# sykefi/syke-pic

Measured on AMD Instinct MI355X. Metric: IFCB images/sec, resnet50 224x224 infer step, higher is better.
Workload: dtype f16

## Files before the change

### syke-pic_amd/csrc/conv_stem.hip

```cpp
#include "spk_common.h"
#include <cstdlib>

namespace {

constexpr int TILE = 16;
constexpr int PH = 2 * TILE + 5;
constexpr int PWP = TILE + 4;
constexpr int PATCH_BYTES = PH * PWP * 16;
constexpr int W_ROW_BYTES = 512;

constexpr int POOL_STEP = 14;
constexpr int POOL_OUT = 7;

template <int DT, int SPLITW, int POOL>
__global__ __launch_bounds__(256) void conv_stem_kernel(ConvArgs a, int tiles_x, int tiles_y, int n_tiles) {
  constexpr int NW = SPLITW ? 2 : 1;
  constexpr int NJ = POOL ? 2 : 4;
  constexpr int WROWS = 16 * NJ;
  constexpr int W_BYTES = WROWS * W_ROW_BYTES;
  const int cb = POOL ? (int)(blockIdx.x & 1) : 0;
  constexpr int EPI_LD = 68;
  constexpr int TSTEP = POOL ? POOL_STEP : TILE;
  constexpr int TORG = POOL ? 1 : 0;
  extern __shared__ __attribute__((aligned(16))) unsigned char smem[];
  unsigned char* const sW = smem;
  unsigned char* const sP = smem + NW * W_BYTES;
  float* const sE = (float*)(sP + 2 * PATCH_BYTES);
  unsigned char* const sH = sP + 2 * PATCH_BYTES;
  constexpr int HSTRIDE = 80;

  const int tid = threadIdx.x, lane = tid & 63;
  const int wave = __builtin_amdgcn_readfirstlane(tid >> 6);
  const int frow = lane & 15, fq = lane >> 4;

  const __amdgpu_buffer_rsrc_t rx = __builtin_amdgcn_make_buffer_rsrc((void*)a.x, 0, a.x_bytes, 0x00020000);

  for (int c = tid; c < NW * WROWS * 32; c += 256) {
    const int ch = c & 31, row = (c >> 5) % WROWS, half = c / (WROWS * 32);
    const int srow = POOL ? 32 * cb + 8 * ((row & 15) >> 2) + 4 * (row >> 4) + (row & 3) : row;
    const u32x4_t v = *(const u32x4_t*)(a.w + ((size_t)(half * 64 + srow) * 256 + ch * 8));
    *(u32x4_t*)(sW + half * W_BYTES + row * W_ROW_BYTES + ((ch ^ (row & 15)) << 4)) = v;
  }

  constexpr int P_IT = (PH * PWP + 255) / 256;
  u32x4_t rp[P_IT];
  auto issue_patch = [&](int tile) {
    const int img = tile / (tiles_x * tiles_y);
    const int rem = tile - img * tiles_x * tiles_y;
    const int ty = rem / tiles_x, tx = rem - ty * tiles_x;
    const int iy0 = (ty * TSTEP - TORG) * 2 - 3, ix0 = (tx * TSTEP - TORG) * 2 - 4;
#pragma unroll
    for (int i = 0; i < P_IT; ++i) {
      const int c = tid + i * 256;
      const int pr = c / PWP, pp = c - pr * PWP;
      const int iy = iy0 + pr, ix = ix0 + 2 * pp;
      const bool ok = c < PH * PWP && (unsigned)iy < (unsigned)a.H && (unsigned)ix < (unsigned)a.W;
      const unsigned off = ok ? (unsigned)((((img * a.H + iy) * a.W) + ix) * 8) : 0x80000000u;
      rp[i] = __builtin_amdgcn_raw_buffer_load_b128(rx, off, 0, 0);
    }
  };
  auto store_patch = [&](int buf) {
#pragma unroll
    for (int i = 0; i < P_IT; ++i) {
      const int c = tid + i * 256;
      if (c < PH * PWP) *(u32x4_t*)(sP + buf * PATCH_BYTES + c * 16) = rp[i];
    }
  };

  const int ecol = (lane & 7) * 8, erow = lane >> 3;
  float sc[8], bi[8], s1[8], s2[8];
#pragma unroll
  for (int j = 0; j < 8; ++j) {
    sc[j] = a.scale ? a.scale[ecol + j] : 1.f;
    bi[j] = a.bias ? a.bias[ecol + j] : 0.f;
    s1[j] = s2[j] = 0.f;
  }
  float* const epi = sE + wave * (16 * EPI_LD);
  float psc[8], pbi[8];
  if (POOL) {
#pragma unroll
    for (int j = 0; j < 8; ++j) {
      psc[j] = a.scale ? a.scale[32 * cb + 8 * fq + j] : 1.f;
      pbi[j] = a.bias ? a.bias[32 * cb + 8 * fq + j] : 0.f;
    }
  }

  const int tstep = POOL ? (int)(gridDim.x >> 1) : (int)gridDim.x;
  int tile = POOL ? (int)(blockIdx.x >> 1) : (int)blockIdx.x;
  int buf = 0;
  if (tile < n_tiles) {
    issue_patch(tile);
    store_patch(0);
  }
  __syncthreads();
  for (; tile < n_tiles; tile += tstep) {
    const int next = tile + tstep;
    if (next < n_tiles) issue_patch(next);

    const int img = tile / (tiles_x * tiles_y);
    const int rem = tile - img * tiles_x * tiles_y;
    const int ty = rem / tiles_x, tx = rem - ty * tiles_x;
    const unsigned char* patch = sP + buf * PATCH_BYTES;

    f32x4_t acc[4][NJ];
#pragma unroll
    for (int i = 0; i < 4; ++i)
#pragma unroll
      for (int j = 0; j < NJ; ++j) acc[i][j] = f32x4_t{0.f, 0.f, 0.f, 0.f};
#pragma unroll
    for (int r = 0; r < 7; ++r) {
      u32x4_t fa[4], fb[NJ], fl[SPLITW ? NJ : 1];
#pragma unroll
      for (int i = 0; i < 4; ++i) {
        const int oy = wave * 4 + i;
        fa[i] = *(const u32x4_t*)(patch + ((2 * oy + r) * PWP + frow + fq) * 16);
      }
#pragma unroll
      for (int j = 0; j < NJ; ++j) {
        const int n = j * 16 + frow;
        fb[j] = *(const u32x4_t*)(sW + n * W_ROW_BYTES + (((r * 4 + fq) ^ (n & 15)) << 4));
        if (SPLITW) fl[j] = *(const u32x4_t*)(sW + W_BYTES + n * W_ROW_BYTES + (((r * 4 + fq) ^ (n & 15)) << 4));
      }
#pragma unroll
      for (int i = 0; i < 4; ++i)
#pragma unroll
        for (int j = 0; j < NJ; ++j) {
          if (POOL) {
            acc[i][j] = mfma16<DT>(fb[j], fa[i], acc[i][j]);
            if (SPLITW) acc[i][j] = mfma16<DT>(fl[j], fa[i], acc[i][j]);
          } else {
            acc[i][j] = mfma16<DT>(fa[i], fb[j], acc[i][j]);
            if (SPLITW) acc[i][j] = mfma16<DT>(fa[i], fl[j], acc[i][j]);
          }
        }
    }

    if (POOL) {
      typedef unsigned short u16x2_t __attribute__((ext_vector_type(2)));
      const int ox = tx * TSTEP - TORG + frow;
#pragma unroll
      for (int i = 0; i < 4; ++i) {
        const int oy = ty * TSTEP - TORG + wave * 4 + i;
        const bool inside = (unsigned)oy < (unsigned)a.Ho && (unsigned)ox < (unsigned)a.Wo;
        {
          u32x4_t ov = {0u, 0u, 0u, 0u};
          float v[8];
#pragma unroll
          for (int r = 0; r < 4; ++r) {
            v[r] = fmaxf(acc[i][0][r] * psc[r] + pbi[r], 0.f);
            v[4 + r] = fmaxf(acc[i][NJ - 1][r] * psc[4 + r] + pbi[4 + r], 0.f);
          }
          if (inside) {
#pragma unroll
            for (int j = 0; j < 4; ++j) ov[j] = pack2<DT>(v[2 * j], v[2 * j + 1]) & 0x7fff7fffu;
          }
          u32x4_t hm;
#pragma unroll
          for (int j = 0; j < 4; ++j) {
            unsigned own = ov[j];
            asm volatile("" : "+v"(own));
            unsigned n1 = (unsigned)__builtin_amdgcn_update_dpp(0, (int)own, 0x101, 0xf, 0xf, true);
            asm volatile("" : "+v"(n1), "+v"(own));
            const u16x2_t t = __builtin_elementwise_max(__builtin_bit_cast(u16x2_t, own), __builtin_bit_cast(u16x2_t, n1));
            unsigned n2 = (unsigned)__builtin_amdgcn_update_dpp(0, (int)n1, 0x101, 0xf, 0xf, true);
            asm volatile("" : "+v"(n2));
            const u16x2_t m = __builtin_elementwise_max(t, __builtin_bit_cast(u16x2_t, n2));
            hm[j] = __builtin_bit_cast(unsigned, m);
          }
          if (!(frow & 1) && frow < 2 * POOL_OUT)
            *(u32x4_t*)(sH + ((wave * 4 + i) * POOL_OUT + (frow >> 1)) * HSTRIDE + 8 * fq * 2) = hm;
        }
      }
    } else
#pragma unroll
    for (int i = 0; i < 4; ++i) {
#pragma unroll
      for (int j = 0; j < NJ; ++j)
#pragma unroll
        for (int rr = 0; rr < 4; ++rr) epi[(fq * 4 + rr) * EPI_LD + j * 16 + frow] = acc[i][j][rr];
      __builtin_amdgcn_wave_barrier();
      const int oy = ty * TSTEP - TORG + wave * 4 + i;
#pragma unroll
      for (int p = 0; p < 2; ++p) {
        const int px = erow + p * 8;
        const int ox = tx * TSTEP - TORG + px;
        const f32x4_t v0 = *(const f32x4_t*)(epi + px * EPI_LD + ecol);
        const f32x4_t v1 = *(const f32x4_t*)(epi + px * EPI_LD + ecol + 4);
        float v[8] = {v0[0], v0[1], v0[2], v0[3], v1[0], v1[1], v1[2], v1[3]};
        const bool inside = (unsigned)oy < (unsigned)a.Ho && (unsigned)ox < (unsigned)a.Wo;
        if (POOL) {
        } else if (inside) {
          if (a.stats) {
#pragma unroll
            for (int j = 0; j < 8; ++j) { s1[j] += v[j]; s2[j] += v[j] * v[j]; }
          }
#pragma unroll
          for (int j = 0; j < 8; ++j) {
            v[j] = v[j] * sc[j] + bi[j];
            if (a.relu) v[j] = fmaxf(v[j], 0.f);
          }
          u32x4_t ov;
#pragma unroll
          for (int j = 0; j < 4; ++j) ov[j] = pack2<DT>(v[2 * j], v[2 * j + 1]);
          *(u32x4_t*)(a.y + (((size_t)img * a.Ho + oy) * a.Wo + ox) * 64 + ecol) = ov;
        }
      }
      __builtin_amdgcn_wave_barrier();
    }

    if (next < n_tiles) store_patch(buf ^ 1);
    __syncthreads();
    if (POOL) {
      for (int it = tid; it < POOL_OUT * POOL_OUT * 4; it += 256) {
        const int chunk = it & 3, pp = it >> 2;
        const int ppy = pp / POOL_OUT, ppx = pp - ppy * POOL_OUT;
        const int py = ty * POOL_OUT + ppy, pxg = tx * POOL_OUT + ppx;
        if (py >= a.pool_ho || pxg >= a.pool_wo) continue;
        u32x4_t mx = {0u, 0u, 0u, 0u};
#pragma unroll
        for (int r = 0; r < 3; ++r) {
          const u32x4_t t = *(const u32x4_t*)(sH + ((2 * ppy + r) * POOL_OUT + ppx) * HSTRIDE + chunk * 16);
#pragma unroll
          for (int j = 0; j < 4; ++j) {
            const unsigned int av = mx[j], bv = t[j];
            const unsigned int lo = max(av & 0xffffu, bv & 0xffffu), hi = max(av >> 16, bv >> 16);
            mx[j] = lo | (hi << 16);
          }
        }
        *(u32x4_t*)(a.pool_y + (((size_t)img * a.pool_ho + py) * a.pool_wo + pxg) * 64 + 32 * cb + chunk * 8) = mx;
      }
      __syncthreads();
    }
    buf ^= 1;
  }

  if (a.stats) {
#pragma unroll
    for (int j = 0; j < 8; ++j)
      for (int d = 8; d < 64; d <<= 1) {
        s1[j] += __shfl_xor(s1[j], d);
        s2[j] += __shfl_xor(s2[j], d);
      }
    float* red = sE;
    __syncthreads();
    if (erow == 0) {
#pragma unroll
      for (int j = 0; j < 8; ++j) {
        red[(wave * 2 + 0) * 64 + ecol + j] = s1[j];
        red[(wave * 2 + 1) * 64 + ecol + j] = s2[j];
      }
    }
    __syncthreads();
    if (tid < 128) {
      const float t = (red[tid] + red[128 + tid]) + (red[256 + tid] + red[384 + tid]);
      a.stats[(size_t)blockIdx.x * 128 + tid] = t;
    }
  }
}

template <int DT, int SPLITW, int POOL>
int launch(const ConvArgs& a, hipStream_t s, int* m_tiles_out) {
  const int tiles_x = POOL ? (a.pool_wo + POOL_OUT - 1) / POOL_OUT : (a.Wo + TILE - 1) / TILE;
  const int tiles_y = POOL ? (a.pool_ho + POOL_OUT - 1) / POOL_OUT : (a.Ho + TILE - 1) / TILE;
  const int n_tiles = a.N * tiles_x * tiles_y;
  const size_t lds = (SPLITW ? 2 : 1) * (POOL ? 32 : 64) * W_ROW_BYTES + 2 * PATCH_BYTES +
                     (POOL ? TILE * POOL_OUT * 80 : 4 * 16 * 68 * 4);
  int grid = 256 * 2;
  if (SPLITW && !POOL) grid = 256;
  if (POOL) {
    if (grid > 2 * n_tiles) grid = 2 * n_tiles;
  } else if (grid > n_tiles) {
    grid = n_tiles;
  }
  auto k = conv_stem_kernel<DT, SPLITW, POOL>;
  static std::atomic<unsigned long long> attr;
  (void)spk_lds_limit_once(attr, (const void*)k, (int)lds);
  if (m_tiles_out) *m_tiles_out = grid;
  hipLaunchKernelGGL(k, dim3(grid), dim3(256), lds, s, a, tiles_x, tiles_y, n_tiles);
  return hipGetLastError() == hipSuccess ? 0 : -1;
}

}

int spk_conv_stem_launch(const ConvArgs& a, hipStream_t s, int* m_tiles_out) {
  if (a.Cout != 64 || a.kh != 7 || a.stride != 2 || a.pad != 3 || a.res) return -2;
  if (a.pool_y) {
    if (!a.relu || a.stats || a.pool_ho != (a.Ho - 1) / 2 + 1 || a.pool_wo != (a.Wo - 1) / 2 + 1) return -2;
    if (a.dt == DT_F16) return a.splitw ? launch<DT_F16, 1, 1>(a, s, m_tiles_out) : launch<DT_F16, 0, 1>(a, s, m_tiles_out);
    return launch<DT_BF16, 0, 1>(a, s, m_tiles_out);
  }
  if (a.dt == DT_F16) return a.splitw ? launch<DT_F16, 1, 0>(a, s, m_tiles_out) : launch<DT_F16, 0, 0>(a, s, m_tiles_out);
  return launch<DT_BF16, 0, 0>(a, s, m_tiles_out);
}
```

Before: 78410.

## Carry pooling halo across stem conv tiles instead of recomputing overlap

Adds a POOL==2 variant of the fused stem conv+maxpool kernel. Each block pair owns whole images and walks tiles in raster order, carrying the left column halo in registers and the top row halo in an LDS buffer. This lets tiles step by the full 16 instead of 14, so the overlapping conv outputs are no longer recomputed. The cost is a grid limited to twice the batch size, which can reduce parallelism for small batches, plus extra LDS that scales with image width. The new path is the default when that halo fits, and an environment variable restores the old tiled path.

```diff
diff --git a/syke-pic_amd/csrc/conv_stem.hip b/syke-pic_amd/csrc/conv_stem.hip
--- a/syke-pic_amd/csrc/conv_stem.hip
+++ b/syke-pic_amd/csrc/conv_stem.hip
@@ -11,6 +11,7 @@
 
 constexpr int POOL_STEP = 14;
 constexpr int POOL_OUT = 7;
+constexpr int HALO_MAX_BYTES = 32 * 1024;
 
 template <int DT, int SPLITW, int POOL>
 __global__ __launch_bounds__(256) void conv_stem_kernel(ConvArgs a, int tiles_x, int tiles_y, int n_tiles) {
@@ -20,14 +21,17 @@
   constexpr int W_BYTES = WROWS * W_ROW_BYTES;
   const int cb = POOL ? (int)(blockIdx.x & 1) : 0;
   constexpr int EPI_LD = 68;
-  constexpr int TSTEP = POOL ? POOL_STEP : TILE;
-  constexpr int TORG = POOL ? 1 : 0;
+  constexpr bool CARRY = POOL == 2;
+  constexpr int PO = CARRY ? 8 : POOL_OUT;
+  constexpr int TSTEP = POOL == 1 ? POOL_STEP : TILE;
+  constexpr int TORG = POOL == 1 ? 1 : 0;
   extern __shared__ __attribute__((aligned(16))) unsigned char smem[];
   unsigned char* const sW = smem;
   unsigned char* const sP = smem + NW * W_BYTES;
   float* const sE = (float*)(sP + 2 * PATCH_BYTES);
   unsigned char* const sH = sP + 2 * PATCH_BYTES;
   constexpr int HSTRIDE = 80;
+  unsigned char* const sR = sH + TILE * PO * HSTRIDE;
 
   const int tid = threadIdx.x, lane = tid & 63;
   const int wave = __builtin_amdgcn_readfirstlane(tid >> 6);
@@ -85,16 +89,26 @@
     }
   }
 
-  const int tstep = POOL ? (int)(gridDim.x >> 1) : (int)gridDim.x;
-  int tile = POOL ? (int)(blockIdx.x >> 1) : (int)blockIdx.x;
+  const int tpi = tiles_x * tiles_y;
+  const int pairs = (int)(gridDim.x >> 1);
+  const int tstep = POOL ? pairs : (int)gridDim.x;
+  int tile = CARRY ? (int)(blockIdx.x >> 1) * tpi : POOL ? (int)(blockIdx.x >> 1) : (int)blockIdx.x;
+  auto next_tile = [&](int t) {
+    if (!CARRY) return t + tstep;
+    const int img = t / tpi;
+    return t + 1 - img * tpi < tpi ? t + 1 : (img + pairs) * tpi;
+  };
+  u32x4_t carry[4];
+#pragma unroll
+  for (int i = 0; i < 4; ++i) carry[i] = u32x4_t{0u, 0u, 0u, 0u};
   int buf = 0;
   if (tile < n_tiles) {
     issue_patch(tile);
     store_patch(0);
   }
   __syncthreads();
-  for (; tile < n_tiles; tile += tstep) {
-    const int next = tile + tstep;
+  for (; tile < n_tiles; tile = next_tile(tile)) {
+    const int next = next_tile(tile);
     if (next < n_tiles) issue_patch(next);
 
     const int img = tile / (tiles_x * tiles_y);
@@ -138,6 +152,10 @@
     if (POOL) {
       typedef unsigned short u16x2_t __attribute__((ext_vector_type(2)));
       const int ox = tx * TSTEP - TORG + frow;
+      if (CARRY && tx == 0) {
+#pragma unroll
+        for (int i = 0; i < 4; ++i) carry[i] = u32x4_t{0u, 0u, 0u, 0u};
+      }
 #pragma unroll
       for (int i = 0; i < 4; ++i) {
         const int oy = ty * TSTEP - TORG + wave * 4 + i;
@@ -155,6 +173,22 @@
             for (int j = 0; j < 4; ++j) ov[j] = pack2<DT>(v[2 * j], v[2 * j + 1]) & 0x7fff7fffu;
           }
           u32x4_t hm;
+          if (CARRY) {
+#pragma unroll
+            for (int j = 0; j < 4; ++j) {
+              unsigned own = ov[j];
+              asm volatile("" : "+v"(own));
+              const unsigned sel = frow == 15 ? carry[i][j] : own;
+              unsigned n1 = (unsigned)__builtin_amdgcn_update_dpp(0, (int)own, 0x101, 0xf, 0xf, true);
+              asm volatile("" : "+v"(n1), "+v"(own));
+              unsigned l1 = (unsigned)__builtin_amdgcn_update_dpp(0, (int)sel, 0x121, 0xf, 0xf, true);
+              asm volatile("" : "+v"(l1), "+v"(own));
+              const u16x2_t t = __builtin_elementwise_max(__builtin_bit_cast(u16x2_t, own), __builtin_bit_cast(u16x2_t, n1));
+              const u16x2_t m = __builtin_elementwise_max(t, __builtin_bit_cast(u16x2_t, l1));
+              hm[j] = __builtin_bit_cast(unsigned, m);
+              carry[i][j] = own;
+            }
+          } else
 #pragma unroll
           for (int j = 0; j < 4; ++j) {
             unsigned own = ov[j];
@@ -167,8 +201,8 @@
             const u16x2_t m = __builtin_elementwise_max(t, __builtin_bit_cast(u16x2_t, n2));
             hm[j] = __builtin_bit_cast(unsigned, m);
           }
-          if (!(frow & 1) && frow < 2 * POOL_OUT)
-            *(u32x4_t*)(sH + ((wave * 4 + i) * POOL_OUT + (frow >> 1)) * HSTRIDE + 8 * fq * 2) = hm;
+          if (!(frow & 1) && frow < 2 * PO)
+            *(u32x4_t*)(sH + ((wave * 4 + i) * PO + (frow >> 1)) * HSTRIDE + 8 * fq * 2) = hm;
         }
       }
     } else
@@ -210,7 +244,32 @@
 
     if (next < n_tiles) store_patch(buf ^ 1);
     __syncthreads();
-    if (POOL) {
+    if (CARRY) {
+      const int chunk = tid & 3, pp = tid >> 2;
+      const int ppy = pp >> 3, ppx = pp & 7;
+      const int py = ty * 8 + ppy, pxg = tx * 8 + ppx;
+      u32x4_t mx = {0u, 0u, 0u, 0u};
+      if (ppy == 0) {
+        unsigned char* const r = sR + (tx * 8 + ppx) * HSTRIDE + chunk * 16;
+        if (ty > 0) mx = *(const u32x4_t*)r;
+        *(u32x4_t*)r = *(const u32x4_t*)(sH + (15 * 8 + ppx) * HSTRIDE + chunk * 16);
+      }
+#pragma unroll
+      for (int r = 0; r < 3; ++r) {
+        const int row = 2 * ppy - 1 + r;
+        if (row < 0) continue;
+        const u32x4_t t = *(const u32x4_t*)(sH + (row * 8 + ppx) * HSTRIDE + chunk * 16);
+#pragma unroll
+        for (int j = 0; j < 4; ++j) {
+          const unsigned int av = mx[j], bv = t[j];
+          const unsigned int lo = max(av & 0xffffu, bv & 0xffffu), hi = max(av >> 16, bv >> 16);
+          mx[j] = lo | (hi << 16);
+        }
+      }
+      if (py < a.pool_ho && pxg < a.pool_wo)
+        *(u32x4_t*)(a.pool_y + (((size_t)img * a.pool_ho + py) * a.pool_wo + pxg) * 64 + 32 * cb + chunk * 8) = mx;
+      __syncthreads();
+    } else if (POOL) {
       for (int it = tid; it < POOL_OUT * POOL_OUT * 4; it += 256) {
         const int chunk = it & 3, pp = it >> 2;
         const int ppy = pp / POOL_OUT, ppx = pp - ppy * POOL_OUT;
@@ -260,21 +319,24 @@
 
 template <int DT, int SPLITW, int POOL>
 int launch(const ConvArgs& a, hipStream_t s, int* m_tiles_out) {
-  const int tiles_x = POOL ? (a.pool_wo + POOL_OUT - 1) / POOL_OUT : (a.Wo + TILE - 1) / TILE;
-  const int tiles_y = POOL ? (a.pool_ho + POOL_OUT - 1) / POOL_OUT : (a.Ho + TILE - 1) / TILE;
+  const int tiles_x = POOL == 1 ? (a.pool_wo + POOL_OUT - 1) / POOL_OUT : (a.Wo + TILE - 1) / TILE;
+  const int tiles_y = POOL == 1 ? (a.pool_ho + POOL_OUT - 1) / POOL_OUT : (a.Ho + TILE - 1) / TILE;
   const int n_tiles = a.N * tiles_x * tiles_y;
-  const size_t lds = (SPLITW ? 2 : 1) * (POOL ? 32 : 64) * W_ROW_BYTES + 2 * PATCH_BYTES +
-                     (POOL ? TILE * POOL_OUT * 80 : 4 * 16 * 68 * 4);
+  const size_t lds_base = (SPLITW ? 2 : 1) * (POOL ? 32 : 64) * W_ROW_BYTES + 2 * PATCH_BYTES +
+                          (POOL ? TILE * (POOL == 2 ? 8 : POOL_OUT) * 80 : 4 * 16 * 68 * 4);
+  const size_t lds = lds_base + (POOL == 2 ? (size_t)tiles_x * 8 * 80 : 0);
   int grid = 256 * 2;
   if (SPLITW && !POOL) grid = 256;
-  if (POOL) {
+  if (POOL == 2) {
+    if (grid > 2 * a.N) grid = 2 * a.N;
+  } else if (POOL) {
     if (grid > 2 * n_tiles) grid = 2 * n_tiles;
   } else if (grid > n_tiles) {
     grid = n_tiles;
   }
   auto k = conv_stem_kernel<DT, SPLITW, POOL>;
   static std::atomic<unsigned long long> attr;
-  (void)spk_lds_limit_once(attr, (const void*)k, (int)lds);
+  (void)spk_lds_limit_once(attr, (const void*)k, (int)(lds_base + (POOL == 2 ? HALO_MAX_BYTES : 0)));
   if (m_tiles_out) *m_tiles_out = grid;
   hipLaunchKernelGGL(k, dim3(grid), dim3(256), lds, s, a, tiles_x, tiles_y, n_tiles);
   return hipGetLastError() == hipSuccess ? 0 : -1;
@@ -286,6 +348,11 @@
   if (a.Cout != 64 || a.kh != 7 || a.stride != 2 || a.pad != 3 || a.res) return -2;
   if (a.pool_y) {
     if (!a.relu || a.stats || a.pool_ho != (a.Ho - 1) / 2 + 1 || a.pool_wo != (a.Wo - 1) / 2 + 1) return -2;
+    static const bool tiled = getenv("SPK_STEM_POOL_TILED") && atoi(getenv("SPK_STEM_POOL_TILED"));
+    if (!tiled && (size_t)(a.Wo + TILE - 1) / TILE * 8 * 80 <= (size_t)HALO_MAX_BYTES) {
+      if (a.dt == DT_F16) return a.splitw ? launch<DT_F16, 1, 2>(a, s, m_tiles_out) : launch<DT_F16, 0, 2>(a, s, m_tiles_out);
+      return launch<DT_BF16, 0, 2>(a, s, m_tiles_out);
+    }
     if (a.dt == DT_F16) return a.splitw ? launch<DT_F16, 1, 1>(a, s, m_tiles_out) : launch<DT_F16, 0, 1>(a, s, m_tiles_out);
     return launch<DT_BF16, 0, 1>(a, s, m_tiles_out);
   }
```

Result: no change. 78530, median of 6 (+0.2%).
